# mpkuse/solve_keyframe_pose_graph

Hardware: AMD Instinct MI355X
Metric: LM iters/sec + final chi2 vs Ceres, 100k-pose/300k-edge SE(3) graph (higher is better)
Workload: dtype f64

## Files before the change

solve_keyframe_pose_graph_amd/_build.py:

```python
import os
import shutil
import subprocess

_HERE = os.path.dirname(os.path.abspath(__file__))
CSRC = os.path.join(_HERE, "csrc")
INCLUDE = os.path.join(os.path.dirname(_HERE), "include")
LIBPGO = os.path.join(_HERE, "libpgo.so")
LIBGEN = os.path.join(_HERE, "libpgo_graphgen.so")

HIP_SOURCES = ["pgo_kernels.hip", "pgo_solver.hip", "pgo_graph.hip", "pgo_shard.hip", "pgo_measure.hip", "pgo_pcg.hip", "pgo_multigrid.hip", "pgo_comm.hip"]
HIP_HEADERS = ["pgo_handle.hpp", "pgo_internal.hpp", "pgo_device_math.hpp", "pgo_mg_kernels.hpp", "pgo_mg_host.hpp", "pgo_comm.hpp"]


def _stale(target, deps):
    if not os.path.exists(target):
        return True
    t = os.path.getmtime(target)
    return any(os.path.exists(d) and os.path.getmtime(d) > t for d in deps)


def hipcc_path():
    for c in (os.environ.get("HIPCC"), shutil.which("hipcc"), "/opt/rocm/bin/hipcc"):
        if c and os.path.exists(c):
            return c
    raise RuntimeError("hipcc not found: libpgo cannot be built (there is no CPU fallback)")


def build_graphgen(force=False):
    src = os.path.join(CSRC, "pgo_graphgen.cpp")
    if force or _stale(LIBGEN, [src, os.path.join(INCLUDE, "pgo_graphgen.h")]):
        subprocess.check_call(["g++", "-O2", "-std=c++17", "-fPIC", "-shared", "-I", INCLUDE, "-o", LIBGEN, src])
    return LIBGEN


HIP_FLAGS = ["--offload-arch=gfx950", "-O3", "-std=c++17", "-fPIC", "-ffp-contract=on"]
_ROOT = os.path.dirname(_HERE)
OBJ_DIR = os.path.join(_ROOT, "build", "obj")


def source_tree_hash(extra_flags=()):
    import hashlib
    h = hashlib.sha256()
    files = [os.path.join(CSRC, f) for f in HIP_SOURCES + HIP_HEADERS] + [os.path.join(INCLUDE, "pgo.h")]
    for f in files:
# ... 80 lines not shown
```

solve_keyframe_pose_graph_amd/csrc/pgo_graph.hip:

```cpp
#include <algorithm>
#include <cstdio>
#include <vector>

#include "pgo_handle.hpp"

namespace {

void meas_from_matrix(const double* T, double w, double* out8) {
    double R[9];
    for (int r = 0; r < 3; ++r) for (int c = 0; c < 3; ++c) R[r * 3 + c] = T[c * 4 + r];
    double q[4];
    eigen_matrix_to_quat(R, q);
    out8[0] = q[0]; out8[1] = q[1]; out8[2] = q[2]; out8[3] = q[3];
    out8[4] = T[12]; out8[5] = T[13]; out8[6] = T[14]; out8[7] = w;
}

struct LocalIndex {
    const int32_t* g2l;
    int32_t operator()(int32_t g) const { return g2l ? g2l[g] : g; }
};

const char* validate(const HostClass& rel, const HostClass& swe, const std::vector<PriorDev>& priors, int64_t N, int64_t S, std::vector<uint8_t>& sw_used) {
    for (const HostClass* H : {&rel, &swe})
        for (int64_t e = 0; e < H->size(); ++e)
            if (H->c1[e] < 0 || H->c1[e] >= N || H->c2[e] < 0 || H->c2[e] >= N) return "edge endpoint out of range for n_nodes";
    sw_used.assign((size_t)S, 0);
    for (int64_t e = 0; e < swe.size(); ++e) {
        const int32_t si = swe.sw[e];
        if (si < 0 || si >= S) return "switch index out of range for n_switch";
        if (sw_used[si]) return "switch index used by more than one edge";
        sw_used[si] = 1;
    }
    for (const PriorDev& pr : priors) if (pr.node < 0 || pr.node >= N) return "regulariser node out of range";
    return nullptr;
}

std::vector<uint8_t> free_flags(const HostClass& rel, const HostClass& swe, const std::vector<PriorDev>& priors, const std::vector<int32_t>& constant_nodes, LocalIndex L,
                                int64_t N, int64_t N_global, const std::vector<int32_t>& l2g, const std::vector<uint8_t>& touched_any) {
    std::vector<uint8_t> touched_here((size_t)N, 0), node_free((size_t)N, 0);
// ... 57 lines not shown
    for (int64_t k = 0; k < Eg; ++k) rowptr[I.priors[k].node + 1]++;
    for (int64_t n = 0; n < N; ++n) rowptr[n + 1] += rowptr[n];
    I.inc.resize((size_t)rowptr[N]); I.bsr_col.resize((size_t)bsr_rowptr[N]);
    std::vector<int64_t> fill(rowptr.begin(), rowptr.end() - 1), bfill(N);
    for (int64_t n = 0; n < N; ++n) { I.bsr_col[bsr_rowptr[n]] = (int32_t)n; bfill[n] = bsr_rowptr[n] + 1; }
    auto add_edge = [&](int64_t slot, int32_t a, int32_t b) {
        I.inc[fill[a]++] = (slot << 1) | 0; I.bsr_col[bfill[a]++] = b;
        I.inc[fill[b]++] = (slot << 1) | 1; I.bsr_col[bfill[b]++] = a;
    };
    for (int64_t e = 0; e < Er; ++e) add_edge(e, L(rel.c1[e]), L(rel.c2[e]));
    for (int64_t e = 0; e < Es; ++e) add_edge(rel_Epad + e, L(swe.c1[e]), L(swe.c2[e]));
    for (int64_t k = 0; k < Eg; ++k) I.inc[fill[I.priors[k].node]++] = ((rel_Epad + sw_Epad + k) << 1);
    return I;
}

bool matrix_free_eligible(const IncidentLists& I, int64_t N, int64_t slot_pr0) {
    for (int64_t n = 0; n < N; ++n) {
        int64_t deg = 0, npri = 0;
        for (int64_t k = I.rowptr[n]; k < I.rowptr[n + 1]; ++k) { if ((I.inc[k] >> 1) >= slot_pr0) ++npri; else ++deg; }
        if (deg > MF_BLOCK || npri > 1) return false;
    }
    return true;
}

struct MfTiles {
    std::vector<int32_t> tile_node0;
    std::vector<int64_t> tile_inc0;
    std::vector<int32_t> tile_sw0;
    std::vector<uint32_t> einc, eslot;
    std::vector<int32_t> eoth;
    std::vector<ushort4> node_rng;
    std::vector<int32_t> node_prior;
    int64_t pair_lanes = 0, rel_side_lanes = 0, sw_lanes = 0;
    int tiles() const { return (int)tile_node0.size() - 1; }
};
const char* pack_mf_tiles(const IncidentLists& I, const HostClass& rel, const HostClass& swe, LocalIndex L, int64_t N, int64_t rel_Epad, int64_t sw_Epad, MfTiles& M) {
    const std::vector<int64_t>& rowptr = I.rowptr; const std::vector<int64_t>& inc = I.inc;
    const int64_t Er = rel.size(), Es = swe.size();
    std::vector<int32_t> deg_rel(N, 0), deg_sw(N, 0);
    M.node_prior.assign(N, -1);
    const int64_t slot_pr = rel_Epad + sw_Epad;
    for (int64_t n = 0; n < N; ++n) {
        for (int64_t k = rowptr[n]; k < rowptr[n + 1]; ++k) {
            const int64_t slot = inc[k] >> 1;
            if (slot >= slot_pr) {
                if (M.node_prior[n] >= 0) return "matrix-free operator: more than one regulariser on a keyframe";
                M.node_prior[n] = (int32_t)(slot - slot_pr);
            } else if (slot >= rel_Epad) ++deg_sw[n]; else ++deg_rel[n];
        }
        if (deg_rel[n] + deg_sw[n] > MF_BLOCK) return "matrix-free operator: a keyframe with more incident edges than a matrix-free tile holds (use PGO_LINEAR_PCG_BLOCK_JACOBI)";
    }
    if ((int64_t)std::max(Er, Es) >= (1ll << 30)) return "matrix-free operator: more than 2^30 edges in one class";
    auto rel_other_of = [&](int64_t k) -> int32_t {
        const int64_t slot = inc[k] >> 1; const int side = (int)(inc[k] & 1);
        if (slot >= rel_Epad) return -1;
        const int32_t a = L(rel.c1[slot]), b = L(rel.c2[slot]);
        return a == b ? -1 : (side == 0 ? b : a);
    };
    std::vector<int32_t>& tile_node0 = M.tile_node0;
    tile_node0.assign(1, 0);
    { int64_t sides = 0, pairs = 0; int cur_nodes = 0; int32_t start = 0;
      for (int64_t n = 0; n < N; ++n) {
          const int64_t d = deg_rel[n] + deg_sw[n];
          auto pairs_with = [&](int32_t lo) { int64_t c = 0; for (int64_t k = rowptr[n]; k < rowptr[n + 1]; ++k) { const int32_t o = rel_other_of(k); if (o >= lo && o < (int32_t)n) ++c; } return c; };
          int64_t np = pairs_with(start);
          if (sides + d > MF_SLOTS || sides + d - (pairs + np) > MF_BLOCK || cur_nodes >= MF_MAX_NODES) {
              tile_node0.push_back((int32_t)n); sides = 0; pairs = 0; cur_nodes = 0; start = (int32_t)n; np = 0;
          }
          sides += d; pairs += np; ++cur_nodes;
      }
      tile_node0.push_back((int32_t)N); }
    const int tiles = M.tiles();
    std::vector<int64_t>& tile_inc0 = M.tile_inc0; std::vector<int32_t>& tile_sw0 = M.tile_sw0;
    std::vector<uint32_t>& einc = M.einc; std::vector<uint32_t>& eslot = M.eslot; std::vector<int32_t>& eoth = M.eoth; std::vector<ushort4>& node_rng = M.node_rng;
    tile_inc0.assign(tiles + 1, 0);
    tile_sw0.assign(std::max(tiles, 1), 0);
    node_rng.resize(std::max<int64_t>(N, 1));
    einc.reserve((size_t)(Er + 2 * Es) + 64); eoth.reserve(einc.capacity()); eslot.reserve(einc.capacity());
    std::vector<uint16_t> side_slot((size_t)(rowptr[N]), 0);
    std::vector<uint16_t> rel_slot1((size_t)std::max<int64_t>(Er, 1), 0);
    for (int t = 0; t < tiles; ++t) {
        const int32_t n0 = tile_node0[t], n1 = tile_node0[t + 1];
        tile_inc0[t] = (int64_t)einc.size();
        int slot_n = 0;
        for (int pass = 0; pass < 2; ++pass)
            for (int32_t n = n0; n < n1; ++n) {
                const unsigned short begin = (unsigned short)slot_n;
                for (int64_t k = rowptr[n]; k < rowptr[n + 1]; ++k) {
                    const int64_t slot = inc[k] >> 1;
                    if (slot >= slot_pr || (int)(slot >= rel_Epad) != pass) continue;
                    side_slot[k] = (uint16_t)slot_n;
                    if (pass == 0 && (inc[k] & 1)) rel_slot1[slot] = (uint16_t)slot_n;
                    ++slot_n;
                }
                if (pass == 0) { node_rng[n].x = begin; node_rng[n].y = (unsigned short)slot_n; } else { node_rng[n].z = begin; node_rng[n].w = (unsigned short)slot_n; }
            }
        int n_pairs = 0;
        for (int group = 0; group < 3; ++group) {
            if (group == 2) tile_sw0[t] = (int32_t)(((int64_t)einc.size() - tile_inc0[t]) | ((int64_t)n_pairs << 16));
            for (int32_t n = n0; n < n1; ++n)
                for (int64_t k = rowptr[n]; k < rowptr[n + 1]; ++k) {
                    const int64_t slot = inc[k] >> 1; const int side = (int)(inc[k] & 1);
                    if (slot >= slot_pr) continue;
                    const bool is_sw = slot >= rel_Epad;
// ... 24 lines not shown
}

int upload_class(pgo_problem* p, const PackedClass& P, DBuf<int32_t>& dc1, DBuf<int32_t>& dc2, DBuf<int32_t>* dsw, DBuf<double>& dmeas, DBuf<int4>& dwin, EdgeClassDev& out) {
    const bool robust = !dsw && !P.loss.empty();
    if (P.Epad > 0) {
        HIPCHK(p, dc1.upload(P.c1, p->st)); HIPCHK(p, dc2.upload(P.c2, p->st)); HIPCHK(p, dmeas.upload(P.meas, p->st)); HIPCHK(p, dwin.upload(P.win, p->st));
        if (dsw) HIPCHK(p, dsw->upload(P.sw, p->st));
        if (robust) { HIPCHK(p, p->d_rloss.upload(P.loss, p->st)); HIPCHK(p, p->d_rlossc.ensure((size_t)P.Epad)); }
        HIPCHK(p, hipStreamSynchronize(p->st));
    }
    out.c1 = dc1.p; out.c2 = dc2.p; out.meas = dmeas.p; out.swidx = dsw ? dsw->p : nullptr; out.win = dwin.p;
    out.E = P.E; out.Epad = P.Epad; out.tiles = P.tiles(); out.J = nullptr;
    out.loss = robust ? p->d_rloss.p : nullptr; out.lossc = robust ? p->d_rlossc.p : nullptr;
    return PGO_OK;
}

int upload_incident_lists(pgo_problem* p, const IncidentLists& I) {
    HIPCHK(p, p->d_inc_rowptr.upload(I.rowptr, p->st)); HIPCHK(p, p->d_bsr_rowptr.upload(I.bsr_rowptr, p->st)); HIPCHK(p, p->d_inc.upload(I.inc, p->st));
    HIPCHK(p, p->d_bsr_col.upload(I.bsr_col, p->st)); HIPCHK(p, p->d_node_free.upload(p->h_node_free, p->st)); HIPCHK(p, p->d_prior.upload(I.priors, p->st));
    HIPCHK(p, hipStreamSynchronize(p->st));
    return PGO_OK;
}

int upload_mf_tiles(pgo_problem* p, const MfTiles& M) {
    const int64_t ninc_e = (int64_t)M.einc.size();
    const int64_t ninc_pad = (ninc_e + 63) / 64 * 64 + 64;
    HIPCHK(p, p->d_einc.upload(M.einc, p->st)); HIPCHK(p, p->d_einc_slot.upload(M.eslot, p->st)); HIPCHK(p, p->d_einc_other.upload(M.eoth, p->st));
    HIPCHK(p, p->d_node_rng.upload(M.node_rng, p->st)); HIPCHK(p, p->d_tile_inc0.upload(M.tile_inc0, p->st)); HIPCHK(p, p->d_tile_node0.upload(M.tile_node0, p->st));
    HIPCHK(p, p->d_tile_sw0.upload(M.tile_sw0, p->st)); HIPCHK(p, p->d_node_prior.upload(M.node_prior, p->st));
    HIPCHK(p, p->d_rec.ensure((size_t)MF_PLANES * ninc_pad)); HIPCHK(p, p->d_lam.ensure(std::max<int64_t>(p->N * 6, 1)));
    HIPCHK(p, hipStreamSynchronize(p->st));
    p->mf_pair_lanes = M.pair_lanes; p->mf_sw_lanes = M.sw_lanes; p->mf_rel_side_lanes = M.rel_side_lanes;
    p->F = MfDev{p->d_einc.p, p->d_einc_other.p, p->d_einc_slot.p, p->d_tile_inc0.p, p->d_tile_sw0.p, p->d_tile_node0.p, p->d_node_rng.p, p->d_node_prior.p,
                 p->d_rec.p, p->d_lam.p, ninc_e, ninc_pad, M.tiles()};
    return PGO_OK;
}

int allocate_work_buffers(pgo_problem* p) {
    const GraphDev& G = p->G;
    const int64_t N = p->N, S = p->S, Es = G.sw.E, Eg = (int64_t)p->priors.size(), slots = G.rel.Epad + G.sw.Epad;
    const bool mf = p->built_mf;
    HIPCHK(p, p->d_Jr.ensure(std::max<int64_t>((int64_t)G.rel.tiles * REL_DOUBLES * TILE, 1)));
    HIPCHK(p, p->d_Js.ensure(std::max<int64_t>((int64_t)G.sw.tiles * SW_DOUBLES * TILE, 1)));
    HIPCHK(p, p->d_Jp.ensure(std::max<int64_t>(Eg * PRIOR_DOUBLES, 1)));
    HIPCHK(p, p->d_Hd_g.ensure(std::max<int64_t>(N * 42, 1)));
    HIPCHK(p, p->d_Hoff.ensure(mf ? 1 : std::max<int64_t>(slots * 36, 1)));
    HIPCHK(p, p->d_c.ensure(std::max<int64_t>(Es * 12, 1))); HIPCHK(p, p->d_hss.ensure(std::max<int64_t>(Es, 1))); HIPCHK(p, p->d_gs.ensure(std::max<int64_t>(Es, 1)));
    HIPCHK(p, p->d_scale_p.ensure(std::max<int64_t>(N * 6, 1))); HIPCHK(p, p->d_diag_p.ensure(std::max<int64_t>(N * 6, 1)));
    HIPCHK(p, p->d_scale_s.ensure(std::max<int64_t>(Es, 1))); HIPCHK(p, p->d_diag_s.ensure(std::max<int64_t>(Es, 1))); HIPCHK(p, p->d_a_inv.ensure(std::max<int64_t>(Es, 1)));
    HIPCHK(p, p->d_val.ensure(mf ? 1 : std::max<int64_t>(p->nnzb * 36, 1))); HIPCHK(p, p->d_Lf.ensure(std::max<int64_t>(N * 24 + 64 * 24, 1))); HIPCHK(p, p->d_Dtot_b.ensure(std::max<int64_t>(N * 42, 1)));
    HIPCHK(p, p->d_cgvec.ensure(std::max<int64_t>(N * 42, 1)));
    p->n_part = std::max<int64_t>(MAX_PARTIALS, (G.rel.tiles + G.sw.tiles + 3) / 4 + 1);
    HIPCHK(p, p->d_part.ensure(p->n_part * 6));
    HIPCHK(p, p->d_cgpart.ensure(PQ_SLOTS + 2 * RZ_STRIDE + 16));
    HIPCHK(p, p->d_flags.ensure(8)); HIPCHK(p, p->d_scal.ensure(S_N));
    for (int k = 0; k < 2; ++k) { HIPCHK(p, p->d_pose[k].ensure(std::max<int64_t>(N * 8, 1))); HIPCHK(p, p->d_swv[k].ensure(std::max<int64_t>(S, 1))); }
    HIPCHK(p, p->d_delta_s.ensure(std::max<int64_t>(Es, 1))); HIPCHK(p, p->d_io.ensure(std::max<int64_t>(N * 7, 1)));
    return PGO_OK;
}
void bind_descriptors(pgo_problem* p) {
    GraphDev& G = p->G;
    const int64_t N = p->N;
    G.rel.J = p->d_Jr.p; G.sw.J = p->d_Js.p;
    G.prior = p->d_prior.p; G.n_prior = (int32_t)p->priors.size(); G.Jp = p->d_Jp.p;
    G.inc_rowptr = p->d_inc_rowptr.p; G.inc = p->d_inc.p; G.node_free = p->d_node_free.p;
    G.bsr_rowptr = p->d_bsr_rowptr.p; G.bsr_col = p->d_bsr_col.p; G.nnzb = p->nnzb;
    p->L = LinDev{p->d_Hd_g.p, p->d_Hd_g.p + (size_t)N * 36, p->d_Hoff.p, p->d_c.p, p->d_hss.p, p->d_gs.p};
// ... 29 lines not shown
    mg_drop_pending(p);
    double t_phase = now_s();
    auto phase = [&](const char* what) { if (p->opt.verbosity > 1) { const double t = now_s(); std::fprintf(stderr, "[pgo] build_graph: %-34s %7.2f ms\n", what, (t - t_phase) * 1e3); t_phase = t; } };
    auto fail = [&](const char* text) { p->err = text; return PGO_ERR_INVALID_ARG; };
    int rc;
    if (const char* bad = validate(p->rel, p->swe, p->priors, N, S, p->h_sw_used)) return fail(bad);
    p->S = S; p->N_global = N;
    GraphDev& G = p->G;
    G = GraphDev{};
    if ((rc = number_rank_local(p, p->N_global, &N)) != PGO_OK) return rc;
    p->N = N;
    phase("validation, rank-local numbering");
    const LocalIndex L{p->local_ids ? p->g2l.data() : nullptr};
    G.N = N; G.S = S;
    p->h_node_free = free_flags(p->rel, p->swe, p->priors, p->constant_nodes, L, N, p->N_global, p->l2g, p->h_touched_any);

    struct Guard { pgo_problem* p; bool committed = false; ~Guard() { if (!committed) mg_drop_pending(p); } } mg_guard{p};
    mg_start_fresh(p, sw_now);
    if ((rc = upload_class(p, pack_class(p->rel, false, L), p->d_rc1, p->d_rc2, nullptr, p->d_rmeas, p->d_rwin, G.rel)) != PGO_OK) return rc;
    if ((rc = upload_class(p, pack_class(p->swe, true, L), p->d_sc1, p->d_sc2, &p->d_sidx, p->d_smeas, p->d_swin, G.sw)) != PGO_OK) return rc;
    phase("edge classes packed + uploaded");

    const IncidentLists I = incident_lists(p->rel, p->swe, p->priors, L, N, G.rel.Epad, G.sw.Epad);
    p->nnzb = I.nnzb();
    if ((rc = upload_incident_lists(p, I)) != PGO_OK) return rc;
    phase("incident lists + block-CSR structure");

    p->built_mf = p->opt.linear_solver == PGO_LINEAR_PCG_MATRIX_FREE && matrix_free_eligible(I, N, G.rel.Epad + G.sw.Epad);
    p->F = MfDev{};
    if (p->built_mf) {
        MfTiles M;
        if (const char* bad = pack_mf_tiles(I, p->rel, p->swe, L, N, G.rel.Epad, G.sw.Epad, M)) return fail(bad);
        if ((rc = upload_mf_tiles(p, M)) != PGO_OK) return rc;
    }
    phase("matrix-free tiles");

    if ((rc = allocate_work_buffers(p)) != PGO_OK) return rc;
    bind_descriptors(p);
    phase("work buffers");

    if ((rc = build_multigrid(p, sw_now)) != PGO_OK) return rc;
    phase("multigrid hierarchy");
    if (p->mg.built && p->built_mf) { HIPCHK(p, p->d_Hoff.ensure((size_t)(p->G.rel.Epad + p->G.sw.Epad) * 36)); p->L.Hoff = p->d_Hoff.p; }
    p->hoff_epoch = 0;
    if (!p->mg.built && (rc = build_two_level_aggregates(p)) != PGO_OK) return rc;
    phase("two-level aggregates");
    mg_guard.committed = true;
    p->graph_dirty = false; p->priors_dirty = false;
    ++p->pcg.build_epoch;
    return PGO_OK;
}

}
```

solve_keyframe_pose_graph_amd/csrc/pgo_handle.hpp:

```cpp
#pragma once
#include <hip/hip_runtime.h>

#include <chrono>
#include <cstdlib>
#include <cstring>
#include <memory>
#include <string>
#include <thread>
#include <vector>

#include "pgo.h"
#include "pgo_internal.hpp"
#include "pgo_comm.hpp"
#include "pgo_mg_host.hpp"

#pragma GCC visibility push(hidden)
namespace pgo {

inline double now_s() { return std::chrono::duration<double>(std::chrono::steady_clock::now().time_since_epoch()).count(); }

inline bool debug_hooks_enabled() { static const bool on = []() { const char* e = std::getenv("PGO_ENABLE_DEBUG_HOOKS"); return e && e[0] == '1' && e[1] == 0; }(); return on; }
inline bool debug_poison() { static const bool on = []() { const char* e = std::getenv("PGO_DEBUG_POISON"); return debug_hooks_enabled() && e && e[0] == '1' && e[1] == 0; }(); return on; }
inline bool debug_break_coarse() { if (!debug_hooks_enabled()) return false; const char* e = std::getenv("PGO_DEBUG_BREAK_COARSE"); return e && e[0] == '1' && e[1] == 0; }

inline bool debug_no_split_update() { static const bool on = []() { const char* e = std::getenv("PGO_DEBUG_NO_SPLIT_UPDATE"); return debug_hooks_enabled() && e && e[0] == '1' && e[1] == 0; }(); return on; }
inline bool debug_split_hosts(int* a, int* b) {
    static const int v = []() {
        const char* e = std::getenv("PGO_DEBUG_SPLIT_HOSTS");
        if (!debug_hooks_enabled() || !e) return -1;
        char* end = nullptr; const long x = std::strtol(e, &end, 10);
        if (!end || *end != ',' || x < 0 || x > 63) return -1;
        const long y = std::strtol(end + 1, &end, 10);
        return (end && *end == 0 && y >= x && y <= 63) ? (int)(x * 64 + y) : -1;
    }();
    if (v < 0) return false;
    *a = v / 64; *b = v % 64;
    return true;
}

inline int debug_graph_after() {
    static const int v = []() {
        const char* e = std::getenv("PGO_DEBUG_GRAPH_AFTER");
        if (!debug_hooks_enabled() || !e) return 192;
        char* end = nullptr; const long n = std::strtol(e, &end, 10);
        return (end && *end == 0 && n >= 2 && n <= 1000000 && (n & 1) == 0) ? (int)n : 192;
    }();
    return v;
}

template <class T>
struct DBuf {
    T* p = nullptr;
    size_t cap = 0;
    DBuf() = default;
    DBuf(const DBuf&) = delete;
    DBuf& operator=(const DBuf&) = delete;
    ~DBuf() { if (p) (void)hipFree(p); }
    hipError_t ensure(size_t n) {
        if (n <= cap) return hipSuccess;
        if (p) { (void)hipFree(p); p = nullptr; cap = 0; }
        const size_t want = n + n / 8 + 64;
        hipError_t e = hipMalloc((void**)&p, want * sizeof(T));
        if (e == hipSuccess) cap = want;
        if (e == hipSuccess && debug_poison()) { e = hipMemset(p, 0xFF, want * sizeof(T)); if (e == hipSuccess) e = hipDeviceSynchronize(); }
        return e;
    }
    hipError_t upload(const std::vector<T>& v, hipStream_t st) {
        hipError_t e = ensure(v.empty() ? 1 : v.size());
        if (e == hipSuccess && !v.empty()) e = hipMemcpyAsync(p, v.data(), v.size() * sizeof(T), hipMemcpyHostToDevice, st);
        return e;
    }
};

struct EventPair {
    hipEvent_t e0 = nullptr, e1 = nullptr;
    hipError_t create() { hipError_t e = hipEventCreate(&e0); if (e == hipSuccess) e = hipEventCreate(&e1); return e; }
    ~EventPair() { if (e0) (void)hipEventDestroy(e0); if (e1) (void)hipEventDestroy(e1); }
};

struct HostClass {
// ... 262 lines not shown
```

solve_keyframe_pose_graph_amd/csrc/pgo_internal.hpp:

```cpp
#pragma once
#include <hip/hip_runtime.h>
#include <stdint.h>

#include "pgo_device_math.hpp"

#define PGO_HIPCHK(err, expr)                                                                      \
    do {                                                                                           \
        hipError_t e__ = (expr);                                                                   \
        if (e__ != hipSuccess) {                                                                   \
            (err) = std::string(#expr) + ": " + hipGetErrorString(e__);                            \
            return e__ == hipErrorOutOfMemory ? PGO_ERR_OUT_OF_MEMORY : PGO_ERR_HIP;               \
        }                                                                                          \
    } while (0)

namespace pgo {

constexpr int TILE = 64;
constexpr int REL_DOUBLES = 78;
constexpr int SW_DOUBLES = 86;
constexpr int K1_WAVES = 4;
constexpr int WIN_MAX = 72;
constexpr int WIN_STRIDE = 80;
constexpr int MAX_PARTIALS = 1024;
constexpr int CG_MAX_GRID = 1024;
constexpr int RZ_STRIDE = CG_MAX_GRID + MAX_PARTIALS;
constexpr int PQ_SLOTS = CG_MAX_GRID;
constexpr int PRIOR_DOUBLES = 42;
constexpr int MF_BLOCK = 256;
constexpr int MF_MAX_NODES = 42;
constexpr int MF_SLOTS = 384;
constexpr int MF_MAX_GRID = 1024;
constexpr int MF_PLANES = 8;

struct PriorDev {
    double Rf[9];
    double tf[3];
    double qf[4];
    double w;
    int32_t node;
    int32_t pad_;
};

struct EdgeClassDev {
    const int32_t* c1;
    const int32_t* c2;
    const double* meas;
    const int32_t* swidx;
    const int4* win;
    double* J;
    int64_t E, Epad;
    int32_t tiles;
    const double* loss;
    double* lossc;
};

struct GraphDev {
    int64_t N, S;
    EdgeClassDev rel, sw;
    const PriorDev* prior; int32_t n_prior; double* Jp;
    const int64_t* inc_rowptr; const int64_t* inc;
    const uint8_t* node_free;
    const double* own;
    const int64_t* bsr_rowptr; const int32_t* bsr_col; int64_t nnzb;
};

struct MfDev {
    const uint32_t* einc;
    const int32_t* einc_other;
    const uint32_t* einc_slot;
    const int64_t* tile_inc0;
    const int32_t* tile_sw0;
    const int32_t* tile_node0;
    const ushort4* node_rng;
    const int32_t* node_prior;
    double2* rec;
    double* lam;
    int64_t ninc, ninc_pad;
    int32_t tiles;
};

struct LinDev {
    double* Hd; double* g; double* Hoff; double* c; double* hss; double* gs;
};

struct ScaleDev {
    double* scale_p;
    double* scale_s;
    double* diag_p;
    double* diag_s;
    double* a_inv;
};

struct CoarseDev {
    int32_t n_agg, nc;
    int32_t m;
    int32_t n_blk;
    double* cen;
    double* d;
    double* Ac;
    double* rc;
    double* yc;
    const int64_t* blk_ptr;
    const int32_t* blk_ab;
    const int64_t* contrib;
    const int32_t* agg_free;
    float* Acf;
};

constexpr int MG_MAX_LEVELS = 12;
constexpr int MG_TILE_ROWS = 32;
struct MgLevelDev {
// ... 157 lines not shown
```

solve_keyframe_pose_graph_amd/csrc/pgo_kernels.hip:

```cpp
#include <algorithm>

#include "pgo_internal.hpp"

namespace pgo {

#ifndef PGO_NO_UNIFORM
__device__ __forceinline__ int wave_in_grid() { return __builtin_amdgcn_readfirstlane((int)(((int64_t)blockIdx.x * blockDim.x + threadIdx.x) >> 6)); }
__device__ __forceinline__ int wave_in_block() { return __builtin_amdgcn_readfirstlane((int)(threadIdx.x >> 6)); }
#else
__device__ __forceinline__ int wave_in_grid() { return (int)(((int64_t)blockIdx.x * blockDim.x + threadIdx.x) >> 6); }
__device__ __forceinline__ int wave_in_block() { return (int)(threadIdx.x >> 6); }
#endif

__device__ __forceinline__ double wave_sum(double v) {
#pragma unroll
    for (int o = 32; o > 0; o >>= 1) v += __shfl_down(v, o, 64);
    return v;
}
__device__ __forceinline__ double wave_max(double v) {
#pragma unroll
    for (int o = 32; o > 0; o >>= 1) v = fmax(v, __shfl_down(v, o, 64));
    return v;
}
#ifndef PGO_SERIAL_HEAD
// ... 1139 lines not shown
    const Pose P2 = load_pose_global(pose8, C.c2[e]);
    const double* mp = C.meas + e;
    const size_t ep = (size_t)C.Epad;
    const Meas M{mp[0], mp[ep], mp[2 * ep], mp[3 * ep], mp[4 * ep], mp[5 * ep], mp[6 * ep], mp[7 * ep]};
    const double ws = is_sw ? swv[C.swidx[e]] : LOSS ? M.w * G.rel.lossc[e] : M.w;
    double rec[COMPACT_DOUBLES];
    edge_compact(P1, P2, M, ws, is_sw, rec);
    for (int pl = 0; pl < MF_PLANES; ++pl) F.rec[(size_t)pl * F.ninc_pad + i] = make_double2(rec[2 * pl], rec[2 * pl + 1]);
}

__device__ __forceinline__ double coarse_pending(const CoarseDev& K, const uint8_t* __restrict__ node_free, int64_t node, int r) {
    const double fr = node_free[node] ? 1.0 : 0.0;
    const double* y = K.yc + (size_t)(node / K.m) * 6;
    const double* d = K.d + (size_t)node * 3;
    const int c = r < 3 ? r : r - 3, c1 = c == 2 ? 0 : c + 1, c2 = c == 0 ? 2 : c - 1;
    const double yr = y[r], ya = y[c1], yb = y[c2], da = d[c1], db = d[c2];
    return fr * (r < 3 ? yr : yr - 2.0 * (da * yb - db * ya));
}

#ifdef PGO_MF_TIMELINE
__device__ unsigned long long pgo_mf_tl[MF_MAX_GRID * 16];
#define MF_TL(slot) do { __builtin_amdgcn_s_waitcnt(0); if (threadIdx.x == 0 && (slot) < 16) pgo_mf_tl[blockIdx.x * 16 + (slot)] = wall_clock64(); } while (0)
extern "C" int pgo_debug_mf_timeline(unsigned long long* out, int n) {
    return (int)hipMemcpyFromSymbol(out, HIP_SYMBOL(pgo_mf_tl), (size_t)n * sizeof(unsigned long long), 0, hipMemcpyDeviceToHost);
}
#else
#define MF_TL(slot) do {} while (0)
#endif

template <bool FUSED, bool COARSE = false>
#ifndef PGO_MF_WAVES
#define PGO_MF_WAVES 1
#endif
__global__ __launch_bounds__(MF_BLOCK, PGO_MF_WAVES) void mf_spmv_kernel(GraphDev G, MfDev F, ScaleDev Sc, CgDev C, const double* __restrict__ xin, double* __restrict__ yout,
                                                           int parity, int first, int nparts, double tol2, CoarseDev K = CoarseDev{}, int pending = 0) {
    __shared__ double contrib[MF_SLOTS * 7];
    __shared__ double pwin[MF_BLOCK];
    __shared__ double red[3 * (MF_BLOCK / 64) + 1];
    const int l = threadIdx.x;
    MF_TL(0);
    double beta = 0.0;
    const double* __restrict__ pprev = FUSED ? (parity ? C.p : C.p2) : xin;
    const double* __restrict__ z = FUSED ? C.z : xin;
    double v0_first = 0.0, v1_first = 0.0;
    int64_t i0_first = 0, i1_first = 0; int32_t n0_first = 0, n1_first = 0, sw_first = 0;
    {
        const int tile = blockIdx.x;
        if (tile < F.tiles) {
            i0_first = F.tile_inc0[tile]; i1_first = F.tile_inc0[tile + 1]; sw_first = F.tile_sw0[tile];
            const int32_t n0 = F.tile_node0[tile], n1 = F.tile_node0[tile + 1];
            n0_first = n0; n1_first = n1;
            if (l < (n1 - n0) * 6) {
                const size_t vi = (size_t)n0 * 6 + l;
                v0_first = z[vi];
                if (FUSED) v1_first = pprev[vi];
                if (COARSE && pending) { const double cp = coarse_pending(K, G.node_free, (int64_t)n0 + l / 6, l % 6); v0_first = K.m == 1 ? cp : v0_first + cp; }
            }
        }
    }
    if (!FUSED && first == 3) { if (cg_done(C)) return; }
    if (FUSED) {
        if (first) { if (cg_done(C)) return; }
        else {
            double rz_new, rz_old;
            bool coarse_negative = false;
            bool stopped;
            if (COARSE) {
                double rz_bj, rz_c;
                stopped = block_total3_done(C.flags, C.part_rz + parity * RZ_STRIDE, nparts, C.part_rz + parity * RZ_STRIDE + nparts, C.extra_rz, C.part_rz + (parity ^ 1) * RZ_STRIDE, nparts + C.extra_rz, red, rz_bj, rz_c, rz_old);
                rz_new = rz_bj + rz_c;
                coarse_negative = K.m != 1 && !(rz_new > C.scal[3] * C.scal[0]) && rz_bj > C.scal[3] * C.scal[0];
            } else stopped = block_total2_done(C.flags, C.part_rz + parity * RZ_STRIDE, nparts + C.extra_rz, C.part_rz + (parity ^ 1) * RZ_STRIDE, nparts + C.extra_rz, red, rz_new, rz_old);
            if (stopped) return;
            const bool breakdown = C.flags[1] != 0;
            if (breakdown || !(rz_new > C.scal[3] * C.scal[0])) {
                if (blockIdx.x == 0 && threadIdx.x == 0) { C.flags[0] = 1; if (!breakdown) { C.scal[1] = rz_new; if (coarse_negative || !(rz_new >= -C.scal[3] * C.scal[0])) C.flags[1] = 1; } }
                return;
            }
            beta = rz_new / rz_old;
            if (blockIdx.x == 0 && threadIdx.x == 0) C.scal[1] = rz_new;
        }
        if (blockIdx.x == 0 && threadIdx.x == 0) C.flags[2] += 1;
    }
    MF_TL(1);
    double* __restrict__ pcur = parity ? C.p2 : C.p;
    double pq = 0.0;
#ifdef PGO_MF_TIMELINE
    int tl_base = 2;
#endif
    for (int tile = blockIdx.x; tile < F.tiles; tile += gridDim.x) {
        const bool is_first = tile == (int)blockIdx.x;
        const int64_t i0 = is_first ? i0_first : F.tile_inc0[tile], i1 = is_first ? i1_first : F.tile_inc0[tile + 1];
        const int32_t n0 = is_first ? n0_first : F.tile_node0[tile], n1 = is_first ? n1_first : F.tile_node0[tile + 1];
        const int32_t swp = is_first ? sw_first : F.tile_sw0[tile];
        const int sw0 = swp & 0xffff, pair1 = (int)((uint32_t)swp >> 16);
        const int64_t i = i0 + l;
        const int nn = n1 - n0;
        MF_TL(tl_base + 0);
        if (l < nn * 6) {
            double v;
            if (COARSE) {
                const size_t vi = (size_t)n0 * 6 + l;
                double zf = v0_first;
                if (tile != (int)blockIdx.x) {
                    zf = z[vi];
                    if (pending) { const double cp = coarse_pending(K, G.node_free, (int64_t)n0 + l / 6, l % 6); zf = K.m == 1 ? cp : zf + cp; }
                }
                v = zf + beta * (tile == (int)blockIdx.x ? v1_first : pprev[vi]);
            } else if (tile == (int)blockIdx.x) v = FUSED ? v0_first + beta * v1_first : v0_first;
            else {
                const size_t vi = (size_t)n0 * 6 + l;
                v = z[vi];
                if (FUSED) v += beta * pprev[vi];
            }
            pwin[l] = v;
        }
        __syncthreads();
        MF_TL(tl_base + 1);
        if (i < i1) {
            const uint32_t ent = F.einc[i];
            const int32_t other = F.einc_other[i];
            const uint32_t sl = F.einc_slot[i];
            const bool is_sw = l >= sw0;
            const int side = (int)(ent & 1u);
            const int ownl = (int)(sl >> 18), slot_a = (int)(sl & 511u), slot_b = (int)((sl >> 9) & 511u);
            double rec[COMPACT_DOUBLES];
#pragma unroll
            for (int pl = 0; pl < 8; ++pl) { const double2 v = F.rec[(size_t)pl * F.ninc_pad + i]; rec[2 * pl] = v.x; rec[2 * pl + 1] = v.y; }
            double kscale = 0.0;
            if (is_sw) {
                {
                    const double q2c[4] = {-rec[0], -rec[1], -rec[2], rec[3]};
                    double dq[4];
                    quat_mul(q2c, rec + 4, dq);
                    rec[16] = rec[11]; rec[17] = rec[12]; rec[18] = rec[13];
                    rec[19] = 2.0 * dq[0]; rec[20] = 2.0 * dq[1]; rec[21] = 2.0 * dq[2];
                }
                kscale = sqrt(Sc.a_inv[(ent & 0x7fffffffu) >> 1]);
            } else {
#pragma unroll
                for (int k = 16; k < COMPACT_DOUBLES; ++k) rec[k] = 0.0;
            }
            MF_TL(tl_base + 2);
            double po[6], pt[6];
            {
                const double* a = pwin + ownl * 6;
#pragma unroll
                for (int c = 0; c < 6; ++c) po[c] = a[c];
// ... 11 lines not shown
#pragma unroll
                        for (int c = 0; c < 6; ++c) pt[c] = 0.0;
                    }
                    {
                        const double fr = G.node_free[other] ? 1.0 : 0.0;
                        const double* yy = K.yc + (size_t)(other / K.m) * 6;
                        const double* dd = K.d + (size_t)other * 3;
                        const double y0 = yy[0], y1 = yy[1], y2 = yy[2], y3 = yy[3], y4 = yy[4], y5 = yy[5], d0 = dd[0], d1 = dd[1], d2 = dd[2];
                        pt[0] += fr * y0; pt[1] += fr * y1; pt[2] += fr * y2;
                        pt[3] += fr * (y3 - 2.0 * (d1 * y2 - d2 * y1));
                        pt[4] += fr * (y4 - 2.0 * (d2 * y0 - d0 * y2));
                        pt[5] += fr * (y5 - 2.0 * (d0 * y1 - d1 * y0));
                    }
                }
                if (FUSED) {
                    const double2* c = reinterpret_cast<const double2*>(pprev + (size_t)other * 6);
                    const double2 c0 = c[0], c1 = c[1], c2 = c[2];
                    pt[0] += beta * c0.x; pt[1] += beta * c0.y; pt[2] += beta * c1.x; pt[3] += beta * c1.y; pt[4] += beta * c2.x; pt[5] += beta * c2.y;
                }
            }
            MF_TL(tl_base + 3);
            double y[6];
            if (l < pair1) {
                double y2[6];
                compact_apply_both(rec, po, pt, 0.0, y, y2);
#pragma unroll
                for (int r = 0; r < 6; ++r) contrib[slot_b * 7 + r] = y2[r];
            } else compact_apply(rec, side, po, pt, kscale, y);
#pragma unroll
            for (int r = 0; r < 6; ++r) contrib[slot_a * 7 + r] = y[r];
        }
        __syncthreads();
        MF_TL(tl_base + 4);
        if (l < nn * 6) {
            const int nl = l / 6, r = l - nl * 6;
            const int64_t node = (int64_t)n0 + nl;
            const size_t vi = (size_t)node * 6 + r;
            const double pr = pwin[l];
            const double lam = F.lam[vi];
            const uint8_t is_free = G.node_free[node];
            const ushort4 rg = F.node_rng[node];
            const int32_t pk = F.node_prior[node];
            double acc = lam * pr;
            MF_TL(tl_base + 5);
            if (is_free) {
                for (int j = rg.x; j < rg.y; ++j) acc += contrib[j * 7 + r];
                for (int j = rg.z; j < rg.w; ++j) acc += contrib[j * 7 + r];
                if (pk >= 0) {
                    const double* Jp = G.Jp + (size_t)pk * PRIOR_DOUBLES + 6;
                    double pn[6];
                    for (int c = 0; c < 6; ++c) pn[c] = pwin[nl * 6 + c];
                    double s = 0.0;
                    for (int ii = 0; ii < 6; ++ii) { double t = 0.0; for (int c = 0; c < 6; ++c) t += Jp[ii * 6 + c] * pn[c]; s += Jp[ii * 6 + r] * t; }
                    acc += s;
                }
            }
            if (FUSED) { pcur[vi] = pr; C.q[vi] = acc; pq += acc * pr; }
            else { yout[vi] = acc; pq += acc * pr; }
        }
        __syncthreads();
        MF_TL(tl_base + 6);
#ifdef PGO_MF_TIMELINE
        tl_base += 7;
#endif
    }
    if (FUSED || first >= 2) {
        const double s = block_sum(pq, red);
        if (threadIdx.x == 0) C.part_pq[blockIdx.x] = s;
    }
}

static inline int mf_grid(const MfDev& F) { const int g = F.tiles < MF_MAX_GRID ? F.tiles : MF_MAX_GRID; return g < 1 ? 1 : g; }
int mf_grid_size(const MfDev& F) { return mf_grid(F); }
void launch_mf_compact(const GraphDev& G, const MfDev& F, const double* pose8, const double* sw, hipStream_t st) {
    if (F.ninc <= 0) return;
    if (G.rel.lossc) hipLaunchKernelGGL(mf_compact_kernel<true>, dim3((unsigned)((F.ninc + 255) / 256)), dim3(256), 0, st, G, F, pose8, sw);
    else hipLaunchKernelGGL(mf_compact_kernel<false>, dim3((unsigned)((F.ninc + 255) / 256)), dim3(256), 0, st, G, F, pose8, sw);
}
void launch_mf_spmv(const GraphDev& G, const MfDev& F, const ScaleDev& Sc, const CgDev& C, int k, double tol2, hipStream_t st) {
    const int g = mf_grid(F);
    hipLaunchKernelGGL((mf_spmv_kernel<true, false>), dim3(g), dim3(MF_BLOCK), 0, st, G, F, Sc, C, (const double*)nullptr, (double*)nullptr, k & 1, k == 0 ? 1 : 0, cg_grid(G), tol2);
}
void launch_mf_spmv_coarse(const GraphDev& G, const MfDev& F, const ScaleDev& Sc, const CgDev& C, const CoarseDev& K, int k, double tol2, int nparts, int pending, hipStream_t st) {
    hipLaunchKernelGGL((mf_spmv_kernel<true, true>), dim3(mf_grid(F)), dim3(MF_BLOCK), 0, st, G, F, Sc, C, (const double*)nullptr, (double*)nullptr, k & 1, k == 0 ? 1 : 0, nparts, tol2, K, pending);
}
void launch_mf_apply_dot(const GraphDev& G, const MfDev& F, const ScaleDev& Sc, const CgDev& C, const double* x, double* y, hipStream_t st) {
    hipLaunchKernelGGL((mf_spmv_kernel<false, false>), dim3(mf_grid(F)), dim3(MF_BLOCK), 0, st, G, F, Sc, C, x, y, 0, 2, 0, 0.0);
}
void launch_mf_apply_dot_live(const GraphDev& G, const MfDev& F, const ScaleDev& Sc, const CgDev& C, hipStream_t st) {
    hipLaunchKernelGGL((mf_spmv_kernel<false, false>), dim3(mf_grid(F)), dim3(MF_BLOCK), 0, st, G, F, Sc, C, (const double*)C.z, C.q, 0, 3, 0, 0.0);
}
void launch_mf_apply(const GraphDev& G, const MfDev& F, const ScaleDev& Sc, const CgDev& C, const double* x, double* y, hipStream_t st) {
    hipLaunchKernelGGL((mf_spmv_kernel<false, false>), dim3(mf_grid(F)), dim3(MF_BLOCK), 0, st, G, F, Sc, C, x, y, 0, 1, 0, 0.0);
}

__global__ __launch_bounds__(256) void model_change_kernel(GraphDev G, LinDev L, ScaleDev Sc, const double* __restrict__ dp, double* __restrict__ ds_out, double* __restrict__ partials) {
    __shared__ double red[4];
    const int wave = threadIdx.x >> 6, lane = threadIdx.x & 63;
    const int tile_g = blockIdx.x * 4 + wave;
    const int ntile = G.rel.tiles + G.sw.tiles;
    double mc = 0.0;
    if (tile_g < ntile) {
        const bool is_sw = tile_g >= G.rel.tiles;
        const int tile = is_sw ? tile_g - G.rel.tiles : tile_g;
        const EdgeClassDev& C = is_sw ? G.sw : G.rel;
// ... 1100 lines not shown
```

Before: 117.3.

## Allow larger matrix-free tiles with two row passes and configurable tile cap

Raises the maximum keyframes per matrix-free tile from 42 to 64 and makes the SpMV kernel handle up to two rows per thread, batching the global loads of both rows before using them. It also makes the grid size a per-graph field, adds a debug override for cap and grid, and raises the launch-bounds occupancy hint for non-coarse variants. The packer is refactored into a header with a precomputed per-keyframe summary. By default the cap stays at CAP_MIN (42), so tile count is unchanged unless the debug env is set; choose_cap exists but is not called. The main default-path changes are the new launch bounds and the restructured row passes, which may add register pressure or loop overhead.

```diff
diff --git a/solve_keyframe_pose_graph_amd/_build.py b/solve_keyframe_pose_graph_amd/_build.py
--- a/solve_keyframe_pose_graph_amd/_build.py
+++ b/solve_keyframe_pose_graph_amd/_build.py
@@ -9,7 +9,7 @@
 LIBGEN = os.path.join(_HERE, "libpgo_graphgen.so")
 
 HIP_SOURCES = ["pgo_kernels.hip", "pgo_solver.hip", "pgo_graph.hip", "pgo_shard.hip", "pgo_measure.hip", "pgo_pcg.hip", "pgo_multigrid.hip", "pgo_comm.hip"]
-HIP_HEADERS = ["pgo_handle.hpp", "pgo_internal.hpp", "pgo_device_math.hpp", "pgo_mg_kernels.hpp", "pgo_mg_host.hpp", "pgo_comm.hpp"]
+HIP_HEADERS = ["pgo_handle.hpp", "pgo_internal.hpp", "pgo_device_math.hpp", "pgo_mg_kernels.hpp", "pgo_mg_host.hpp", "pgo_comm.hpp", "pgo_mf_pack.hpp"]
 
 
 def _stale(target, deps):
diff --git a/solve_keyframe_pose_graph_amd/csrc/pgo_graph.hip b/solve_keyframe_pose_graph_amd/csrc/pgo_graph.hip
--- a/solve_keyframe_pose_graph_amd/csrc/pgo_graph.hip
+++ b/solve_keyframe_pose_graph_amd/csrc/pgo_graph.hip
@@ -3,8 +3,11 @@
 #include <vector>
 
 #include "pgo_handle.hpp"
+#include "pgo_mf_pack.hpp"
 
 namespace {
+
+static_assert(pgo_mf_pack::CAP_MAX == MF_MAX_NODES && MF_MAX_NODES * 6 <= MF_SLOTS && pgo_mf_pack::CAP_MIN * 6 <= MF_BLOCK, "the matvec's row passes (mf_spmv_kernel)");
 
 void meas_from_matrix(const double* T, double w, double* out8) {
     double R[9];
@@ -128,6 +131,7 @@
     std::vector<ushort4> node_rng;
     std::vector<int32_t> node_prior;
     int64_t pair_lanes = 0, rel_side_lanes = 0, sw_lanes = 0;
+    int cap = pgo_mf_pack::CAP_MIN, grid = MF_MAX_GRID;
     int tiles() const { return (int)tile_node0.size() - 1; }
 };
 const char* pack_mf_tiles(const IncidentLists& I, const HostClass& rel, const HostClass& swe, LocalIndex L, int64_t N, int64_t rel_Epad, int64_t sw_Epad, MfTiles& M) {
@@ -147,25 +151,18 @@
         if (deg_rel[n] + deg_sw[n] > MF_BLOCK) return "matrix-free operator: a keyframe with more incident edges than a matrix-free tile holds (use PGO_LINEAR_PCG_BLOCK_JACOBI)";
     }
     if ((int64_t)std::max(Er, Es) >= (1ll << 30)) return "matrix-free operator: more than 2^30 edges in one class";
-    auto rel_other_of = [&](int64_t k) -> int32_t {
+    std::vector<int32_t> pack_other((size_t)rowptr[N]);
+    for (int64_t k = 0; k < rowptr[N]; ++k) {
         const int64_t slot = inc[k] >> 1; const int side = (int)(inc[k] & 1);
-        if (slot >= rel_Epad) return -1;
+        if (slot >= rel_Epad) { pack_other[k] = slot >= slot_pr ? pgo_mf_pack::OTHER_NONE : pgo_mf_pack::OTHER_SIDE; continue; }
         const int32_t a = L(rel.c1[slot]), b = L(rel.c2[slot]);
-        return a == b ? -1 : (side == 0 ? b : a);
-    };
+        pack_other[k] = a == b ? pgo_mf_pack::OTHER_SIDE : (side == 0 ? b : a);
+    }
+    const pgo_mf_pack::Keyframes kf(rowptr.data(), pack_other.data(), N);
+    M.grid = MF_MAX_GRID;
+    if (!debug_mf_tiles(&M.cap, &M.grid)) M.cap = pgo_mf_pack::CAP_MIN;
     std::vector<int32_t>& tile_node0 = M.tile_node0;
-    tile_node0.assign(1, 0);
-    { int64_t sides = 0, pairs = 0; int cur_nodes = 0; int32_t start = 0;
-      for (int64_t n = 0; n < N; ++n) {
-          const int64_t d = deg_rel[n] + deg_sw[n];
-          auto pairs_with = [&](int32_t lo) { int64_t c = 0; for (int64_t k = rowptr[n]; k < rowptr[n + 1]; ++k) { const int32_t o = rel_other_of(k); if (o >= lo && o < (int32_t)n) ++c; } return c; };
-          int64_t np = pairs_with(start);
-          if (sides + d > MF_SLOTS || sides + d - (pairs + np) > MF_BLOCK || cur_nodes >= MF_MAX_NODES) {
-              tile_node0.push_back((int32_t)n); sides = 0; pairs = 0; cur_nodes = 0; start = (int32_t)n; np = 0;
-          }
-          sides += d; pairs += np; ++cur_nodes;
-      }
-      tile_node0.push_back((int32_t)N); }
+    pgo_mf_pack::count_tiles(kf, MF_SLOTS, MF_BLOCK, M.cap, &tile_node0);
     const int tiles = M.tiles();
     std::vector<int64_t>& tile_inc0 = M.tile_inc0; std::vector<int32_t>& tile_sw0 = M.tile_sw0;
     std::vector<uint32_t>& einc = M.einc; std::vector<uint32_t>& eslot = M.eslot; std::vector<int32_t>& eoth = M.eoth; std::vector<ushort4>& node_rng = M.node_rng;
@@ -256,7 +253,7 @@
     HIPCHK(p, hipStreamSynchronize(p->st));
     p->mf_pair_lanes = M.pair_lanes; p->mf_sw_lanes = M.sw_lanes; p->mf_rel_side_lanes = M.rel_side_lanes;
     p->F = MfDev{p->d_einc.p, p->d_einc_other.p, p->d_einc_slot.p, p->d_tile_inc0.p, p->d_tile_sw0.p, p->d_tile_node0.p, p->d_node_rng.p, p->d_node_prior.p,
-                 p->d_rec.p, p->d_lam.p, ninc_e, ninc_pad, M.tiles()};
+                 p->d_rec.p, p->d_lam.p, ninc_e, ninc_pad, M.tiles(), M.grid};
     return PGO_OK;
 }
 
@@ -352,6 +349,7 @@
         MfTiles M;
         if (const char* bad = pack_mf_tiles(I, p->rel, p->swe, L, N, G.rel.Epad, G.sw.Epad, M)) return fail(bad);
         if ((rc = upload_mf_tiles(p, M)) != PGO_OK) return rc;
+        if (p->opt.verbosity > 1) std::fprintf(stderr, "[pgo] build_graph: %d matrix-free tiles of <= %d keyframes on <= %d workgroups\n", M.tiles(), M.cap, M.grid);
     }
     phase("matrix-free tiles");
 
diff --git a/solve_keyframe_pose_graph_amd/csrc/pgo_handle.hpp b/solve_keyframe_pose_graph_amd/csrc/pgo_handle.hpp
--- a/solve_keyframe_pose_graph_amd/csrc/pgo_handle.hpp
+++ b/solve_keyframe_pose_graph_amd/csrc/pgo_handle.hpp
@@ -46,6 +46,18 @@
         return (end && *end == 0 && n >= 2 && n <= 1000000 && (n & 1) == 0) ? (int)n : 192;
     }();
     return v;
+}
+
+inline bool debug_mf_tiles(int* keyframes, int* grid) {
+    if (!debug_hooks_enabled()) return false;
+    const char* e = std::getenv("PGO_DEBUG_MF_TILES");
+    if (!e) return false;
+    char* end = nullptr; const long c = std::strtol(e, &end, 10);
+    if (!end || end == e || *end != ',' || c < 1 || c > MF_MAX_NODES) return false;
+    const char* e2 = end + 1; const long g = std::strtol(e2, &end, 10);
+    if (!end || end == e2 || *end != 0 || g < 1 || g > MF_MAX_GRID) return false;
+    *keyframes = (int)c; *grid = (int)g;
+    return true;
 }
 
 template <class T>
diff --git a/solve_keyframe_pose_graph_amd/csrc/pgo_internal.hpp b/solve_keyframe_pose_graph_amd/csrc/pgo_internal.hpp
--- a/solve_keyframe_pose_graph_amd/csrc/pgo_internal.hpp
+++ b/solve_keyframe_pose_graph_amd/csrc/pgo_internal.hpp
@@ -27,7 +27,7 @@
 constexpr int PQ_SLOTS = CG_MAX_GRID;
 constexpr int PRIOR_DOUBLES = 42;
 constexpr int MF_BLOCK = 256;
-constexpr int MF_MAX_NODES = 42;
+constexpr int MF_MAX_NODES = 64;
 constexpr int MF_SLOTS = 384;
 constexpr int MF_MAX_GRID = 1024;
 constexpr int MF_PLANES = 8;
@@ -77,6 +77,7 @@
     double* lam;
     int64_t ninc, ninc_pad;
     int32_t tiles;
+    int32_t grid;
 };
 
 struct LinDev {
diff --git a/solve_keyframe_pose_graph_amd/csrc/pgo_kernels.hip b/solve_keyframe_pose_graph_amd/csrc/pgo_kernels.hip
--- a/solve_keyframe_pose_graph_amd/csrc/pgo_kernels.hip
+++ b/solve_keyframe_pose_graph_amd/csrc/pgo_kernels.hip
@@ -1195,10 +1195,10 @@
 #ifndef PGO_MF_WAVES
 #define PGO_MF_WAVES 1
 #endif
-__global__ __launch_bounds__(MF_BLOCK, PGO_MF_WAVES) void mf_spmv_kernel(GraphDev G, MfDev F, ScaleDev Sc, CgDev C, const double* __restrict__ xin, double* __restrict__ yout,
+__global__ __launch_bounds__(MF_BLOCK, (FUSED && COARSE) ? PGO_MF_WAVES : PGO_MF_WAVES > 4 ? PGO_MF_WAVES : 4) void mf_spmv_kernel(GraphDev G, MfDev F, ScaleDev Sc, CgDev C, const double* __restrict__ xin, double* __restrict__ yout,
                                                            int parity, int first, int nparts, double tol2, CoarseDev K = CoarseDev{}, int pending = 0) {
     __shared__ double contrib[MF_SLOTS * 7];
-    __shared__ double pwin[MF_BLOCK];
+    __shared__ double pwin[MF_SLOTS];
     __shared__ double red[3 * (MF_BLOCK / 64) + 1];
     const int l = threadIdx.x;
     MF_TL(0);
@@ -1260,23 +1260,32 @@
         const int64_t i = i0 + l;
         const int nn = n1 - n0;
         MF_TL(tl_base + 0);
-        if (l < nn * 6) {
-            double v;
+        static_assert(MF_MAX_NODES * 6 <= 2 * MF_BLOCK, "two row passes");
+        const int rows = nn * 6;
+        const bool row_a = l < rows, row_b = l + MF_BLOCK < rows;
+        {
+            struct P0 { double z, pp, cp; };
+            auto request = [&](int ll) {
+                const size_t vi = (size_t)n0 * 6 + ll;
+                P0 o{z[vi], (FUSED || COARSE) ? pprev[vi] : 0.0, 0.0};
+                if (COARSE && pending) o.cp = coarse_pending(K, G.node_free, (int64_t)n0 + ll / 6, ll % 6);
+                return o;
+            };
+            auto value = [&](const P0& o) {
+                double zf = o.z;
+                if (COARSE) { if (pending) zf = K.m == 1 ? o.cp : zf + o.cp; return zf + beta * o.pp; }
+                return FUSED ? zf + beta * o.pp : zf;
+            };
+            auto first_value = [&]() { return (FUSED || COARSE) ? v0_first + beta * v1_first : v0_first; };
             if (COARSE) {
-                const size_t vi = (size_t)n0 * 6 + l;
-                double zf = v0_first;
-                if (tile != (int)blockIdx.x) {
-                    zf = z[vi];
-                    if (pending) { const double cp = coarse_pending(K, G.node_free, (int64_t)n0 + l / 6, l % 6); zf = K.m == 1 ? cp : zf + cp; }
-                }
-                v = zf + beta * (tile == (int)blockIdx.x ? v1_first : pprev[vi]);
-            } else if (tile == (int)blockIdx.x) v = FUSED ? v0_first + beta * v1_first : v0_first;
-            else {
-                const size_t vi = (size_t)n0 * 6 + l;
-                v = z[vi];
-                if (FUSED) v += beta * pprev[vi];
-            }
-            pwin[l] = v;
+                for (int ll = l; ll < rows; ll += MF_BLOCK) pwin[ll] = is_first && ll == l ? first_value() : value(request(ll));
+            } else {
+                P0 a{}, b{};
+                if (row_a && !is_first) a = request(l);
+                if (row_b) b = request(l + MF_BLOCK);
+                if (row_a) pwin[l] = is_first ? first_value() : value(a);
+                if (row_b) pwin[l + MF_BLOCK] = value(b);
+            }
         }
         __syncthreads();
         MF_TL(tl_base + 1);
@@ -1354,31 +1363,42 @@
         }
         __syncthreads();
         MF_TL(tl_base + 4);
-        if (l < nn * 6) {
-            const int nl = l / 6, r = l - nl * 6;
-            const int64_t node = (int64_t)n0 + nl;
-            const size_t vi = (size_t)node * 6 + r;
-            const double pr = pwin[l];
-            const double lam = F.lam[vi];
-            const uint8_t is_free = G.node_free[node];
-            const ushort4 rg = F.node_rng[node];
-            const int32_t pk = F.node_prior[node];
-            double acc = lam * pr;
-            MF_TL(tl_base + 5);
-            if (is_free) {
-                for (int j = rg.x; j < rg.y; ++j) acc += contrib[j * 7 + r];
-                for (int j = rg.z; j < rg.w; ++j) acc += contrib[j * 7 + r];
-                if (pk >= 0) {
-                    const double* Jp = G.Jp + (size_t)pk * PRIOR_DOUBLES + 6;
-                    double pn[6];
-                    for (int c = 0; c < 6; ++c) pn[c] = pwin[nl * 6 + c];
-                    double s = 0.0;
-                    for (int ii = 0; ii < 6; ++ii) { double t = 0.0; for (int c = 0; c < 6; ++c) t += Jp[ii * 6 + c] * pn[c]; s += Jp[ii * 6 + r] * t; }
-                    acc += s;
+        {
+            struct PB { double lam; uint8_t is_free; ushort4 rg; int32_t pk; };
+            auto request = [&](int ll) {
+                const int64_t node = (int64_t)n0 + ll / 6;
+                return PB{F.lam[(size_t)n0 * 6 + ll], G.node_free[node], F.node_rng[node], F.node_prior[node]};
+            };
+            auto finish = [&](int ll, const PB& o) {
+                const int nl = ll / 6, r = ll - nl * 6;
+                const size_t vi = (size_t)n0 * 6 + ll;
+                const double pr = pwin[ll];
+                double acc = o.lam * pr;
+                if (o.is_free) {
+                    for (int j = o.rg.x; j < o.rg.y; ++j) acc += contrib[j * 7 + r];
+                    for (int j = o.rg.z; j < o.rg.w; ++j) acc += contrib[j * 7 + r];
+                    if (o.pk >= 0) {
+                        const double* Jp = G.Jp + (size_t)o.pk * PRIOR_DOUBLES + 6;
+                        double pn[6];
+                        for (int c = 0; c < 6; ++c) pn[c] = pwin[nl * 6 + c];
+                        double s = 0.0;
+                        for (int ii = 0; ii < 6; ++ii) { double t = 0.0; for (int c = 0; c < 6; ++c) t += Jp[ii * 6 + c] * pn[c]; s += Jp[ii * 6 + r] * t; }
+                        acc += s;
+                    }
                 }
-            }
-            if (FUSED) { pcur[vi] = pr; C.q[vi] = acc; pq += acc * pr; }
-            else { yout[vi] = acc; pq += acc * pr; }
+                if (FUSED) { pcur[vi] = pr; C.q[vi] = acc; pq += acc * pr; }
+                else { yout[vi] = acc; pq += acc * pr; }
+            };
+            if (COARSE) {
+                for (int ll = l; ll < rows; ll += MF_BLOCK) finish(ll, request(ll));
+            } else {
+                PB a{}, b{};
+                if (row_a) a = request(l);
+                if (row_b) b = request(l + MF_BLOCK);
+                MF_TL(tl_base + 5);
+                if (row_a) finish(l, a);
+                if (row_b) finish(l + MF_BLOCK, b);
+            }
         }
         __syncthreads();
         MF_TL(tl_base + 6);
@@ -1392,7 +1412,7 @@
     }
 }
 
-static inline int mf_grid(const MfDev& F) { const int g = F.tiles < MF_MAX_GRID ? F.tiles : MF_MAX_GRID; return g < 1 ? 1 : g; }
+static inline int mf_grid(const MfDev& F) { const int g = F.tiles < F.grid ? F.tiles : F.grid; return g < 1 ? 1 : g; }
 int mf_grid_size(const MfDev& F) { return mf_grid(F); }
 void launch_mf_compact(const GraphDev& G, const MfDev& F, const double* pose8, const double* sw, hipStream_t st) {
     if (F.ninc <= 0) return;
diff --git a/solve_keyframe_pose_graph_amd/csrc/pgo_mf_pack.hpp b/solve_keyframe_pose_graph_amd/csrc/pgo_mf_pack.hpp
--- /dev/null
+++ b/solve_keyframe_pose_graph_amd/csrc/pgo_mf_pack.hpp
@@ -0,0 +1,56 @@
+#pragma once
+#include <cstddef>
+#include <cstdint>
+#include <vector>
+
+namespace pgo_mf_pack {
+
+constexpr int CAP_MIN = 42;
+constexpr int CAP_MAX = 64;
+
+constexpr int32_t OTHER_SIDE = -1, OTHER_NONE = -2;
+
+struct Keyframes {
+    const int64_t* rowptr; const int32_t* other; int64_t N;
+    std::vector<int32_t> sides;
+    std::vector<int32_t> back;
+    std::vector<int32_t> back_min;
+    Keyframes(const int64_t* rowptr_, const int32_t* other_, int64_t N_) : rowptr(rowptr_), other(other_), N(N_), sides((size_t)N_), back((size_t)N_), back_min((size_t)N_) {
+        for (int64_t n = 0; n < N; ++n) {
+            int32_t d = 0, nb = 0, mn = (int32_t)n;
+            for (int64_t k = rowptr[n]; k < rowptr[n + 1]; ++k) { const int32_t o = other[k]; if (o != OTHER_NONE) ++d; if (o >= 0 && o < (int32_t)n) { ++nb; if (o < mn) mn = o; } }
+            sides[n] = d; back[n] = nb; back_min[n] = mn;
+        }
+    }
+};
+
+inline int64_t count_tiles(const Keyframes& K, int slots, int lanes, int cap, std::vector<int32_t>* tile_node0 = nullptr) {
+    if (tile_node0) tile_node0->assign(1, 0);
+    int64_t tiles = 1, sides = 0, pairs = 0; int cur_nodes = 0; int32_t start = 0;
+    for (int64_t n = 0; n < K.N; ++n) {
+        const int64_t d = K.sides[n];
+        int64_t np = K.back[n];
+        if (K.back_min[n] < start) { np = 0; for (int64_t k = K.rowptr[n]; k < K.rowptr[n + 1]; ++k) { const int32_t o = K.other[k]; if (o >= start && o < (int32_t)n) ++np; } }
+        if (sides + d > slots || sides + d - (pairs + np) > lanes || cur_nodes >= cap) {
+            if (tile_node0) tile_node0->push_back((int32_t)n);
+            ++tiles; sides = 0; pairs = 0; cur_nodes = 0; start = (int32_t)n; np = 0;
+        }
+        sides += d; pairs += np; ++cur_nodes;
+    }
+    if (tile_node0) tile_node0->push_back((int32_t)K.N);
+    return tiles;
+}
+
+inline int choose_cap(const Keyframes& K, int slots, int lanes, int grid) {
+    auto T = [&](int c) { return count_tiles(K, slots, lanes, c); };
+    if (grid < 1) grid = 1;
+    const int64_t t_min = T(CAP_MIN);
+    if (t_min <= grid) return CAP_MIN;
+    const int64_t room = (T(CAP_MAX) + grid - 1) / grid * grid;
+    if (t_min <= room) return CAP_MIN;
+    int lo = CAP_MIN + 1, hi = CAP_MAX;
+    while (lo < hi) { const int mid = (lo + hi) / 2; if (T(mid) <= room) hi = mid; else lo = mid + 1; }
+    return hi;
+}
+
+}
```

Measured after the change: 117.4 (median of 6 runs). Within noise of the previous version (+0.1%).
